# JiehongLin/SAM-6D

Measured on NVIDIA H100. Metric: poses/sec, higher is better.
Workload: dtype bf16

## Files before the change

include/sam6d_b200.h:

```cpp
#ifndef SAM6D_B200_H
#define SAM6D_B200_H

#ifdef __cplusplus
extern "C" {
#endif


int sam6d_fps(const float* xyz, int b, int n, int m, float* temp, int* idx, void* stream);
int sam6d_fps_single_cta(const float* xyz, int b, int n, int m, float* temp, int* idx, void* stream);

int sam6d_gather_points(const float* points, const int* idx, int b, int c, int n, int m, float* out, void* stream);

int sam6d_gather_rows(const float* src, const int* idx, int b, int n, int m, int c, long long src_bstride, float* out,
                      void* stream);
int sam6d_gather_rows_bf16_f32(const void* src, const int* idx, int b, int n, int m, int c, long long src_bstride, float* out,
                               void* stream);

int sam6d_ball_query(const float* new_xyz, const float* xyz, int b, int n, int m, float radius, int nsample, int* idx,
                     int* cnt, void* stream);
int sam6d_ball_query_pair(const float* new_xyz, const float* xyz, int b, int n, int m, float radius_a, int nsample_a,
                          float radius_b, int nsample_b, int* idx_a, int* idx_b, int* cnt_a, int* cnt_b, void* stream);

int sam6d_group_points(const float* points, const int* idx, int b, int c, int n, int np, int ns, float* out, void* stream);

// ... 43 lines not shown
                        const float* bias, float* E, void* stream);

int sam6d_geo_embed_tc(const float* T, long long npairs, const float* div_term, const void* Wa_bf16, const void* Wd_bf16,
                       const float* bias, void* E, int e_is_bf16, void* stream);
int sam6d_geo_embed_dist_tc(const float* T, long long npairs, const float* div_term, const void* Wd_bf16, const float* bias, void* E,
                            void* stream);
int sam6d_geo_embed_lut(const float* T, long long clouds, int S, const void* tabA, int na, float inv_ha, const void* tabD, int nd,
                        float inv_hd, const void* far, const float* div_term, const void* WdT_bf16, const float* bias, void* E,
                        int precise, void* stream);


int sam6d_inputs_stage_a(const int* rle_cum, const int* rle_off, int P, int H, int W, const float* depth, double fx, double fy,
                         double cx, double cy, double thr, unsigned char* mask, int* stats, int cap, int* choose1, int* choose2,
                         float* cloud2, void* stream);
int sam6d_inputs_stage_b(const int* stats, const int* keep, int Q, int H, int W, int cap, const int* choose2, const float* cloud2,
                         const int* choose_idx, int ns, int S, const unsigned char* image, const unsigned char* mask, int mask_flag,
                         float* pts, long long* rgb_choose, float* rgb, unsigned char* rgb_u8, void* stream);

int sam6d_crop_resize_normalize(const unsigned char* images, const unsigned char* masks, const int* bbox, int Q, int H, int W, int S,
                                int mask_flag, float* rgb, unsigned char* rgb_u8, void* stream);


int sam6d_crop_resize_pad(const unsigned char* image, const float* masks, const int* boxes, int P, int H, int W, int T, float* rgb,
                          float* pmask, void* stream);
int sam6d_masked_patch_normalize(const float* tokens, long long tok_ld, long long tok_bs, const float* pmask, int P, int G, int patch,
                                 int C, float thresh, float* out_f32, void* out_bf16, unsigned char* valid, void* stream);
int sam6d_appearance_reduce(const float* sim, long long sim_ld, long long sim_bs, int P, int N, const unsigned char* qvalid, float thred,
                            float* appe, float* vis, void* stream);


int sam6d_query_translation(const float* masks, const int* depth, int N, int H, int W, const double* K, double depth_scale,
                            float* translate, void* stream);
int sam6d_project_template_iou(const float* poses, int T, const float* pointcloud, int O, int npc, const long long* best_pose,
                               const long long* pred_obj, const float* translate, const double* K, int N, int H, int W,
                               const long long* boxes, int* image_vu, int* xyxy, float* iou, unsigned char* ok, void* stream);


int sam6d_sam_pe_encode(const float* coords, const float* G, int rows, float* out, void* stream);
int sam6d_sam_self_attn(const float* q, const float* k, const float* v, int B, int T, float* out, void* stream);
int sam6d_sam_tok2img_attn(const float* Q, const void* K, const void* V, long long kv_bs, int B, int T, int L, float* out, void* stream);
int sam6d_sam_img2tok_attn(const void* Q, long long q_bs, const float* Kt, const float* Vt, int B, int T, int L, void* out, void* stream);
int sam6d_sam_ln2d_gelu(const void* x, const float* gamma, const float* beta, long long rows, void* y, void* stream);
int sam6d_sam_mask_dot(const void* up, const float* hyper, int B, int G, float* masks, void* stream);
int sam6d_sam_mask_stats(const float* low, int N, int S, int big, int in_h, int in_w, int H, int W, float thr, float off, int* stats,
                         void* stream);
int sam6d_sam_mask_binarize(const float* low, const int* sel, int K, int S, int big, int in_h, int in_w, int H, int W, float thr,
                            unsigned char* out, void* stream);
int sam6d_sam_nms(const float* boxes, int N, float thr, unsigned char* keep, void* stream);


int sam6d_transformer_tail_bf16(const void* hid, long long ld_hid, const void* x, long long ld_x, const void* Wo, const float* bo,
                                const float* g1, const float* b1, const void* We, const float* be, const void* Ws, const float* bs,
                                const float* g2, const float* b2, void* out, long long ld_out, int M, float eps, void* stream);


int sam6d_rpe_scores(const void* E, int e_is_bf16, const float* U, long long u_ld, int B, int S, float* SP, void* stream);
int sam6d_rpe_scores_tc(const void* E, const void* U, int B, int S, float* SP, void* stream);
int sam6d_rpe_scores_tc_ld(const void* E, const void* U, int B, int S, float* SP, int sp_ld, void* stream);
int sam6d_mha(const float* Q, long long q_ld, long long q_bs, const float* K, long long k_ld, long long k_bs, const float* V,
              long long v_ld, long long v_bs, const float* bias, int B, int H, int Sq, int Sk, float scale, float* O,
              long long o_ld, long long o_bs, void* stream);
int sam6d_attn_tc(const void* Q, long long q_ld, int q_col0, const void* K, long long k_ld, int k_col0, const void* Vt,
                  long long vt_ld, int B, int H, int Sq, int Sk, int head_dim, int bias_mode, const float* bias,
                  const void* rel_h, const float* rel_w, int Hs, int Ws, const float* bv, float scale, void* out,
                  int out_is_bf16, long long out_ld, void* stream);
int sam6d_attn_tc_bias_ld(const void* Q, long long q_ld, int q_col0, const void* K, long long k_ld, int k_col0, const void* Vt,
                          long long vt_ld, int B, int H, int Sq, int Sk, int head_dim, const float* bias, long long bias_ld,
                          float scale, void* out, int out_is_bf16, long long out_ld, void* stream);
int sam6d_attn_tc_ex(const void* Q, long long q_ld, int q_col0, const void* K, long long k_ld, int k_col0, const void* Vt,
                     long long vt_ld, int B, int H, int Sq, int Sk, int head_dim, float scale, int k_brows, int k_row0, int v_col0,
                     float* lse, void* out, int out_is_bf16, long long out_ld, void* stream);
int sam6d_attn_merge_key(const void* Q, long long q_ld, int q_col0, const void* K, long long k_ld, int k_col0, int k_brows,
                         int key_row, const void* Vt, long long vt_ld, int key_col, const float* lse, int B, int H, int Sq,
                         float scale, void* out, long long out_ld, void* stream);
int sam6d_transpose_tokens_bf16(const void* src, long long ld, int col0, int C, int nB, int L, int N1, void* out, void* stream);
int sam6d_linattn_kv(const float* Kf, long long k_ld, long long k_bs, const float* V, long long v_ld, long long v_bs, int B,
                     int H, int J, float* KV, float* KS, void* stream);
int sam6d_linattn_apply(const float* Qf, long long q_rpb, long long q_bs, long long q_ld, const float* KV, const float* KS,
                        int B, int H, float* X, long long x_bs, long long x_ld, void* stream);
int sam6d_linattn_kv_pack(const float* Kf, long long k_ld, long long k_bs, const float* V, long long v_ld, long long v_bs, int B,
                          int J, void* blob, float* KS, void* stream);
int sam6d_linattn_tc(const void* Q, long long q_ld, long long q_bs, const void* blob, const float* KS,
                     const float* softplus_scale, int B, int rpb, void* X, long long x_ld, long long x_bs, void* stream);

int sam6d_coarse_assign(const float* A, int B, int S, float* W, float* w1, void* stream);
int sam6d_coarse_sample(const float* W, int B, int L, const float* rand, int nr, int* idx, void* stream);
int sam6d_coarse_hypotheses(const int* idx, const float* pts1, const float* pts2, int B, int n, int n1, float* Rt,
                            float* resid, void* stream);
int sam6d_topk_smallest(const float* v, int B, int n, int k, int* out, void* stream);
int sam6d_coarse_select(const float* Rt, const int* top, int B, int n1, int n2, const float* pts1, const float* w1, int n,
                        const float* model, int nm, float* scores, float* R, float* t, void* stream);


int sam6d_pe_mlp_max(const float* pts, const int* idx, const int* cnt, int B, int N, int ns, const float* W1,
                     const float* B1, const float* W2, const float* B2, const float* W3, const float* B3, float* out,
                     int out_ld, int out_off, void* stream);
int sam6d_pe_mlp_max_tc(const float* pts, const int* idx, int B, int N, int ns, const float* W1, const float* B1,
                        const void* W2_bf16, const float* B2, const void* W3_bf16, const float* B3, void* out, int out_is_bf16,
                        int out_ld, int out_off, void* stream);
int sam6d_fine_assign(const float* A, int B, int S, int ld, float shift, const float* pts2, float* rsum, float* csum, float* cpart,
                      int* cpi, int* lab1, int* lab2, float* wts, float* pred, void* stream);
int sam6d_fine_pass_tc(const void* Fa, const void* Fb, int B, int S, float alpha, float shift, int mode, const float* row_f,
                       const float* col_f, int ld_f, const float* q4, float* out_inv, int* lab, float* wts, float* pred, void* stream);
int sam6d_fine_masked_points(const int* lab2, const float* pts2, int B, int S, int ld, float* q4, void* stream);
int sam6d_weighted_procrustes(const float* src, const float* ref, const float* wts, int B, int N, float weight_thresh,
                              float eps, float* R, float* t, void* stream);
int sam6d_pose_score(const float* pts1, const int* lab1, int B, int N, const float* R, const float* t, const float* model,
                     int nm, float dis_thres, const float* radius, float* score, float* t_scaled, void* stream);

int sam6d_bilinear_gather(const void* up, int up_is_bf16, const long long* choose, int B, int K, int G, int sub, int C, int H, int W,
                          float* out, void* stream);

int sam6d_attn_relpos(const float* qkv, long long tok_ld, int nW, int Hs, int Ws, int nH, int head_dim, const float* rel_h,
                      const float* rel_w, float scale, void* out, int out_is_bf16, long long out_ld, void* stream);

int sam6d_attn_global_tc(const void* qkv, long long ld, const void* Vt, long long vt_ld, const void* rel_blob, int B, int H, int grid,
                         float scale, void* out, int out_is_bf16, long long out_ld, void* stream);

int sam6d_template_score(const float* Qn, const float* Rn, int P, int O, int T, int C, float* sim_out, float* obj_score,
                         int* best_obj, float* best_score, int* best_tmpl, void* stream);

const char* sam6d_version(void);

#ifdef __cplusplus
}
#endif
#endif
```

sam6d_b200/ops.py:

```python
import ctypes
from typing import Optional, Tuple

import torch

from . import _lib

Tensor = torch.Tensor


def _check(t: Tensor, dtype, name: str, ndim: Optional[int] = None):
    if not isinstance(t, torch.Tensor):
        raise RuntimeError(f"{name} must be a torch.Tensor")
    if not t.is_cuda:
        raise RuntimeError(f"{name} must be a CUDA tensor (CPU not supported)")
    if t.dtype != dtype:
        raise RuntimeError(f"{name} must be {dtype}, got {t.dtype}")
    if not t.is_contiguous():
        raise RuntimeError(f"{name} must be contiguous")
    if ndim is not None and t.dim() != ndim:
        raise RuntimeError(f"{name} must have {ndim} dims, got {t.dim()}")


def _p(t: Optional[Tensor]):
    return ctypes.c_void_p(0 if t is None else t.data_ptr())
# ... 466 lines not shown

def attn_global_tc(qkv: Tensor, vt: Tensor, rel_blob: Tensor, B: int, H: int, grid: int, scale: float, out_dtype=torch.bfloat16) -> Tensor:
    _check(qkv, torch.bfloat16, "qkv", 2)
    _check(vt, torch.bfloat16, "vt", 2)
    _check(rel_blob, torch.bfloat16, "rel_blob", 1)
    L = grid * grid
    out = torch.empty(B * L, H * 80, dtype=out_dtype, device=qkv.device)
    _lib.call("sam6d_attn_global_tc", _p(qkv), _ll(qkv.shape[1]), _p(vt), _ll(vt.shape[1]), _p(rel_blob), int(B), int(H), int(grid),
              _f(scale), _p(out), int(out_dtype == torch.bfloat16), _ll(H * 80), _s())
    return out


def attn_tc(Q: Tensor, q_col0: int, K: Tensor, k_col0: int, Vt: Tensor, B: int, H: int, Sq: int, Sk: int, D: int, scale: float,
            bias: Optional[Tensor] = None, rel: Optional[tuple] = None, bv: Optional[Tensor] = None,
            out_dtype=torch.float32, bias_variant: int = 1) -> Tensor:
    _check(Q, torch.bfloat16, "Q", 2)
    _check(K, torch.bfloat16, "K", 2)
    _check(Vt, torch.bfloat16, "Vt", 2)
    mode, rh, rw, Hs, Ws = 0, None, None, 0, 0
    if bias is not None:
        _check(bias, torch.float32, "bias", 4)
        mode = bias_variant
    elif rel is not None:
        rh, Hs, Ws = rel
        mode = 2
    out = torch.empty(B * Sq, H * D, dtype=out_dtype, device=Q.device)
    _lib.call("sam6d_attn_tc", _p(Q), _ll(Q.shape[1]), int(q_col0), _p(K), _ll(K.shape[1]), int(k_col0), _p(Vt), _ll(Vt.shape[1]),
              int(B), int(H), int(Sq), int(Sk), int(D), mode, _p(bias), _p(rh), _p(rw), int(Hs), int(Ws), _p(bv), _f(scale), _p(out),
              int(out_dtype == torch.bfloat16), _ll(H * D), _s())
    return out


def attn_tc_ex(Q: Tensor, q_col0: int, K: Tensor, k_col0: int, Vt: Tensor, B: int, H: int, Sq: int, Sk: int, D: int, scale: float,
               k_brows: int, k_row0: int = 0, v_col0: int = 0, want_lse: bool = False, out_dtype=torch.bfloat16):
    _check(Q, torch.bfloat16, "Q", 2)
    _check(K, torch.bfloat16, "K", 2)
    _check(Vt, torch.bfloat16, "Vt", 2)
    out = torch.empty(B * Sq, H * D, dtype=out_dtype, device=Q.device)
    lse = torch.empty(B, H, Sq, dtype=torch.float32, device=Q.device) if want_lse else None
    _lib.call("sam6d_attn_tc_ex", _p(Q), _ll(Q.shape[1]), int(q_col0), _p(K), _ll(K.shape[1]), int(k_col0), _p(Vt), _ll(Vt.shape[1]),
              int(B), int(H), int(Sq), int(Sk), int(D), _f(scale), int(k_brows), int(k_row0), int(v_col0), _p(lse), _p(out),
              int(out_dtype == torch.bfloat16), _ll(H * D), _s())
    return out, lse


def attn_merge_key(Q: Tensor, q_col0: int, K: Tensor, k_col0: int, k_brows: int, key_row: int, Vt: Tensor, key_col: int, lse: Tensor,
                   B: int, H: int, Sq: int, scale: float, out: Tensor) -> Tensor:
    _check(out, torch.bfloat16, "out", 2)
    _check(lse, torch.float32, "lse", 3)
    _lib.call("sam6d_attn_merge_key", _p(Q), _ll(Q.shape[1]), int(q_col0), _p(K), _ll(K.shape[1]), int(k_col0), int(k_brows), int(key_row),
              _p(Vt), _ll(Vt.shape[1]), int(key_col), _p(lse), int(B), int(H), int(Sq), _f(scale), _p(out), _ll(out.shape[1]), _s())
    return out


def transpose_tokens(src: Tensor, col0: int, C: int, nB: int, L: int) -> Tensor:
    _check(src, torch.bfloat16, "src", 2)
    N1 = (L + 15) // 16 * 16
    out = torch.empty(nB * C, N1, dtype=torch.bfloat16, device=src.device)
    _lib.call("sam6d_transpose_tokens_bf16", _p(src), _ll(src.shape[1]), int(col0), int(C), int(nB), int(L), int(N1), _p(out), _s())
    return out


def linattn_kv_raw(k_ptr, k_ld, k_bs, v_ptr, v_ld, v_bs, B, H, J, KV: Tensor, KS: Tensor):
    _lib.call("sam6d_linattn_kv", ctypes.c_void_p(k_ptr), _ll(k_ld), _ll(k_bs), ctypes.c_void_p(v_ptr), _ll(v_ld), _ll(v_bs),
              int(B), int(H), int(J), _p(KV), _p(KS), _s())


def linattn_apply_raw(q_ptr, q_rpb, q_bs, q_ld, KV: Tensor, KS: Tensor, B, H, x_ptr, x_bs, x_ld):
    _lib.call("sam6d_linattn_apply", ctypes.c_void_p(q_ptr), _ll(q_rpb), _ll(q_bs), _ll(q_ld), _p(KV), _p(KS), int(B), int(H),
              ctypes.c_void_p(x_ptr), _ll(x_bs), _ll(x_ld), _s())


def linattn_kv_pack_raw(k_ptr, k_ld, k_bs, v_ptr, v_ld, v_bs, B, J, device):
    blob = torch.empty(B, 4 * 64 * 64, dtype=torch.bfloat16, device=device)
    KS = torch.empty(B, 4, 64, dtype=torch.float32, device=device)
    _lib.call("sam6d_linattn_kv_pack", ctypes.c_void_p(k_ptr), _ll(k_ld), _ll(k_bs), ctypes.c_void_p(v_ptr), _ll(v_ld), _ll(v_bs),
              int(B), int(J), _p(blob), _p(KS), _s())
    return blob, KS


def linattn_tc_raw(q_ptr, q_ld, q_bs, blob: Tensor, KS: Tensor, sp_scale: Tensor, B, rpb, x_ptr, x_ld, x_bs):
    _lib.call("sam6d_linattn_tc", ctypes.c_void_p(q_ptr), _ll(q_ld), _ll(q_bs), _p(blob), _p(KS), _p(sp_scale), int(B), int(rpb),
              ctypes.c_void_p(x_ptr), _ll(x_ld), _ll(x_bs), _s())


def coarse_assign(A: Tensor) -> Tuple[Tensor, Tensor]:
    _check(A, torch.float32, "atten", 3)
    B, S, _ = A.shape
    n = S - 1
    W = torch.empty(B, n * n, dtype=torch.float32, device=A.device)
    w1 = torch.empty(B, n, dtype=torch.float32, device=A.device)
    _lib.call("sam6d_coarse_assign", _p(A), B, S, _p(W), _p(w1), _s())
    return W, w1


def coarse_sample(W: Tensor, rand: Tensor) -> Tensor:
    _check(W, torch.float32, "W", 2)
    _check(rand, torch.float32, "rand", 2)
    B, L = W.shape
    nr = rand.shape[1]
    idx = torch.empty(B, nr, dtype=torch.int32, device=W.device)
    _lib.call("sam6d_coarse_sample", _p(W), B, L, _p(rand), nr, _p(idx), _s())
    return idx


def coarse_hypotheses(idx: Tensor, pts1: Tensor, pts2: Tensor) -> Tuple[Tensor, Tensor]:
    _check(idx, torch.int32, "idx", 2)
    _check(pts1, torch.float32, "pts1", 3)
    _check(pts2, torch.float32, "pts2", 3)
    B, n, _ = pts1.shape
    n1 = idx.shape[1] // 3
    Rt = torch.empty(B, n1, 12, dtype=torch.float32, device=idx.device)
    resid = torch.empty(B, n1, dtype=torch.float32, device=idx.device)
    _lib.call("sam6d_coarse_hypotheses", _p(idx), _p(pts1), _p(pts2), B, n, n1, _p(Rt), _p(resid), _s())
    return Rt, resid


def topk_smallest(v: Tensor, k: int) -> Tensor:
    _check(v, torch.float32, "v", 2)
    B, n = v.shape
    out = torch.empty(B, k, dtype=torch.int32, device=v.device)
    _lib.call("sam6d_topk_smallest", _p(v), B, n, int(k), _p(out), _s())
    return out


def coarse_select(Rt: Tensor, top: Tensor, pts1: Tensor, w1: Tensor, model: Tensor):
    _check(Rt, torch.float32, "Rt", 3)
    _check(top, torch.int32, "top", 2)
    _check(model, torch.float32, "model", 3)
    B, n1, _ = Rt.shape
    n2 = top.shape[1]
    n = pts1.shape[1]
    scores = torch.empty(B, n2, dtype=torch.float32, device=Rt.device)
    R = torch.empty(B, 3, 3, dtype=torch.float32, device=Rt.device)
    t = torch.empty(B, 3, dtype=torch.float32, device=Rt.device)
    _lib.call("sam6d_coarse_select", _p(Rt), _p(top), B, n1, n2, _p(pts1), _p(w1), n, _p(model), model.shape[1], _p(scores),
              _p(R), _p(t), _s())
    return R, t, scores


def pe_mlp_max(pts: Tensor, idx: Tensor, cnt: Tensor, weights, out: Tensor, out_off: int):
    _check(pts, torch.float32, "pts", 3)
    _check(idx, torch.int32, "idx", 3)
    _check(cnt, torch.int32, "cnt", 2)
    B, N, _ = pts.shape
    ns = idx.shape[2]
    W1, B1, W2, B2, W3, B3 = weights
    _lib.call("sam6d_pe_mlp_max", _p(pts), _p(idx), _p(cnt), B, N, ns, _p(W1), _p(B1), _p(W2), _p(B2), _p(W3), _p(B3),
              _p(out), out.shape[-1], int(out_off), _s())


def pe_mlp_max_tc(pts: Tensor, idx: Tensor, weights, out: Tensor, out_off: int):
    _check(pts, torch.float32, "pts", 3)
    _check(idx, torch.int32, "idx", 3)
    B, N, _ = pts.shape
    ns = idx.shape[2]
    W1, B1, W2, B2, W3, B3 = weights
    _check(W2, torch.bfloat16, "W2", 2)
    _check(W3, torch.bfloat16, "W3", 2)
    if out.dtype not in (torch.float32, torch.bfloat16):
        raise RuntimeError("pe_mlp_max_tc: out must be float32 or bfloat16")
    _lib.call("sam6d_pe_mlp_max_tc", _p(pts), _p(idx), B, N, ns, _p(W1), _p(B1), _p(W2), _p(B2), _p(W3), _p(B3), _p(out),
              int(out.dtype == torch.bfloat16), out.shape[-1], int(out_off), _s())


def fine_assign(A: Tensor, pts2: Tensor, shift: float):
# ... 118 lines not shown
```

sam6d_b200/pem.py:

```python
import math
import os
from types import SimpleNamespace
from typing import Dict, Optional

import torch
import torch.nn as nn

from . import ops

NUM_HEADS = 4

PRECISIONS = ("fp32", "bf16")
FUSED_TAIL = os.environ.get("SAM6D_FUSED_TAIL", "1") != "0"
PADDED_BIAS = os.environ.get("SAM6D_PADDED_BIAS", "1") != "0"
RPE_TC = os.environ.get("SAM6D_RPE_TC", "1") != "0"
GEO_LUT = os.environ.get("SAM6D_GEO_LUT", "1") != "0"
GEO_LUT_PRECISE = os.environ.get("SAM6D_GEO_LUT_PRECISE", "1") != "0"
GEO_LUT_INV_H = 8.0
GEO_LUT_D_MAX = 32.0


class _W:
    __slots__ = ("f32", "bf16")

    def __init__(self, w: torch.Tensor):
        self.f32 = w.detach().to(torch.float32).contiguous()
        self.bf16 = self.f32.to(torch.bfloat16).contiguous()


def _gemm(prec, A, W: "_W", bias=None, residual=None, relu=False):
    if prec == "bf16":
        if A.dtype == torch.bfloat16 and residual is None and A.is_contiguous() and A.shape[1] % 64 == 0:
            return ops.gemm_tma(A, W.bf16, bias, act=1 if relu else 0)
        return ops.gemm_tc(A, W.bf16, bias, residual=residual, relu=relu)
    return ops.gemm(A, W.f32, bias, residual=residual, relu=relu)


def _gemm_raw(prec, A_ptr, W: "_W", bias, R_ptr, C_ptr, M, N, K, lda, ldc, ldr=0, batch=1, sA=0, sC=0, sR=0):
    if prec == "bf16":
        ops.gemm_tc_raw(A_ptr, 0, W.bf16.data_ptr(), 1, bias, R_ptr, C_ptr, 0, M, N, K, lda, K, ldc, ldr, batch=batch, sA=sA, sW=0,
                        sC=sC, sR=sR)
    else:
        ops.gemm_raw(A_ptr, W.f32.data_ptr(), bias, R_ptr, C_ptr, M, N, K, lda, K, ldc, ldr, batch=batch, sA=sA, sW=0, sC=sC, sR=sR)


def _cfg(cfg, **defaults):
    if isinstance(cfg, dict):
        cfg = SimpleNamespace(**cfg)
    for k, v in defaults.items():
        if not hasattr(cfg, k):
            setattr(cfg, k, v)
    return cfg


class _MHAParams(nn.Module):
    def __init__(self, d_model, rpe: bool):
        super().__init__()
        self.proj_q = nn.Linear(d_model, d_model)
        self.proj_k = nn.Linear(d_model, d_model)
        self.proj_v = nn.Linear(d_model, d_model)
        if rpe:
            self.proj_p = nn.Linear(d_model, d_model)


class _AttentionLayerParams(nn.Module):
    def __init__(self, d_model, rpe: bool):
        super().__init__()
        self.attention = _MHAParams(d_model, rpe)
        self.linear = nn.Linear(d_model, d_model)
        self.norm = nn.LayerNorm(d_model)


class _AttentionOutputParams(nn.Module):
    def __init__(self, d_model):
        super().__init__()
        self.expand = nn.Linear(d_model, d_model * 2)
        self.squeeze = nn.Linear(d_model * 2, d_model)
        self.norm = nn.LayerNorm(d_model)


class _TransformerLayerParams(nn.Module):
    def __init__(self, d_model, rpe: bool):
        super().__init__()
        self.attention = _AttentionLayerParams(d_model, rpe)
        self.output = _AttentionOutputParams(d_model)


class _Packed:

    def __init__(self):
        self.key = None
        self.w = {}


def _param_key(module: nn.Module):
    return tuple((p.data_ptr(), p._version) for p in module.parameters()) + tuple(
# ... 450 lines not shown
                ops.pe_mlp_max_tc(pts, idx, w[name + "_tc"], feat, off)
            else:
                ops.pe_mlp_max(pts, idx, cnt, w[name], feat, off)
        return feat

    @torch.no_grad()
    def forward(self, pts1, pts2=None):
        if pts2 is not None and pts2 is not pts1:
            raise NotImplementedError("SAM-6D always calls PE(pts) with a single cloud")
        w = self._weights()
        feat = self.local_features(pts1)
        B, N, _ = feat.shape
        if self.precision == "bf16":
            return ops.gemm_tma(feat.view(B * N, 256), w["w3"].bf16, w["b3"]).view(B, N, -1)
        return _gemm(self.precision, feat.view(B * N, 256), w["w3"], w["b3"]).view(B, N, -1)


class _LinearAttentionParams(nn.Module):
    def __init__(self, d_model):
        super().__init__()
        self.proj_q = nn.Linear(d_model, d_model)
        self.proj_k = nn.Linear(d_model, d_model)
        self.proj_v = nn.Linear(d_model, d_model)
        self.scale = nn.Parameter(torch.zeros(size=(1, 1, d_model)))


class _LinearAttentionLayerParams(nn.Module):
    def __init__(self, d_model):
        super().__init__()
        self.attention = _LinearAttentionParams(d_model)
        self.linear = nn.Linear(d_model, d_model)
        self.norm = nn.LayerNorm(d_model)


class _LinearTransformerLayerParams(nn.Module):
    def __init__(self, d_model):
        super().__init__()
        self.attention = _LinearAttentionLayerParams(d_model)
        self.output = _AttentionOutputParams(d_model)


class SparseToDenseTransformer(nn.Module):

    def __init__(self, d_model, sparse_blocks, num_heads=4, dropout=None, activation_fn='ReLU', parallel=False,
                 focusing_factor=3, with_bg_token=True, replace_bg_token=True):
        super().__init__()
        if not (with_bg_token and replace_bg_token) or focusing_factor != 3:
            raise ValueError("sam6d_b200 SparseToDenseTransformer is built for the SAM-6D configuration")
        self.d_model = d_model
        self.sparse_layer = GeometricTransformer(blocks=sparse_blocks, d_model=d_model, num_heads=num_heads, dropout=dropout,
                                                 activation_fn=activation_fn, parallel=parallel, return_attention_scores=False)
        self.dense_layer = _LinearTransformerLayerParams(d_model)
        self._packed = _Packed()
        self.precision = "fp32"

    def _weights(self):
        key = _param_key(self.dense_layer)
        if self._packed.key != key:
            la = self.dense_layer.attention.attention
            tail = dict(wo=_W(self.dense_layer.attention.linear.weight), bo=_f32(self.dense_layer.attention.linear.bias),
                        g1=_f32(self.dense_layer.attention.norm.weight), b1=_f32(self.dense_layer.attention.norm.bias),
                        we=_W(self.dense_layer.output.expand.weight), be=_f32(self.dense_layer.output.expand.bias),
                        ws=_W(self.dense_layer.output.squeeze.weight), bs=_f32(self.dense_layer.output.squeeze.bias),
                        g2=_f32(self.dense_layer.output.norm.weight), b2=_f32(self.dense_layer.output.norm.bias))
            self._packed.w = dict(
                wq=_W(la.proj_q.weight), bq=_f32(la.proj_q.bias),
                wkv=_W(torch.cat([_f32(la.proj_k.weight), _f32(la.proj_v.weight)], dim=0)),
                bkv=torch.cat([_f32(la.proj_k.bias), _f32(la.proj_v.bias)], dim=0).contiguous(),
                sp_scale=torch.nn.functional.softplus(_f32(la.scale)).reshape(-1).contiguous(), tail=tail)
            self._packed.key = key
        return self._packed.w

    def _sample_feats(self, dense_feats, idx_ext):
        if dense_feats.dtype == torch.bfloat16:
            return ops.gather_rows_bf16(dense_feats, idx_ext)
        return ops.gather_rows(dense_feats, idx_ext)

    def _dense_layer_bf16(self, dense, sparse, w):
        B, N1, C = dense.shape
        N, J = N1 - 1, sparse.shape[1] - 1
        dev = dense.device
        bf = torch.bfloat16
        x2d = dense.view(B * N1, C)
        q = ops.gemm_tma(x2d, w["wq"].bf16, w["bq"], out_dtype=bf)
        kv = torch.empty(B * J, 2 * C, dtype=torch.float32, device=dev)
        s_bf = sparse.dtype == torch.bfloat16
        ops.gemm_tc_raw(sparse.data_ptr() + C * (2 if s_bf else 4), int(s_bf), w["wkv"].bf16.data_ptr(), 1, w["bkv"], 0, kv.data_ptr(), 0,
                        J, 2 * C, C, C, C, 2 * C, 0, batch=B, sA=(J + 1) * C, sW=0, sC=J * 2 * C)
        ops.focus_rows_raw(kv.data_ptr(), (B * J, 0, 2 * C), kv.data_ptr(), (B * J, 0, 2 * C), w["sp_scale"], B * J, C)
        blob, KS = ops.linattn_kv_pack_raw(kv.data_ptr(), 2 * C, J * 2 * C, kv.data_ptr() + C * 4, 2 * C, J * 2 * C, B, J, dev)
        x_att = torch.empty(B * N1, C, dtype=bf, device=dev)
        ops.linattn_tc_raw(q.data_ptr() + C * 2, C, N1 * C, blob, KS, w["sp_scale"], B, N, x_att.data_ptr() + C * 2, C, N1 * C)
        x_att.view(B, N1, C)[:, 0, :] = 0
        t = w["tail"]
        if FUSED_TAIL:
            out = ops.transformer_tail_bf16(x_att, x2d, t["wo"].bf16, t["bo"], t["g1"], t["b1"], t["we"].bf16, t["be"], t["ws"].bf16,
                                            t["bs"], t["g2"], t["b2"]).view(B, N1, C)
        else:
            y = ops.gemm_tma(x_att, t["wo"].bf16, t["bo"], residual=x2d, out_dtype=bf)
            y = ops.layernorm_bf16io(y, t["g1"], t["b1"])
            h = ops.gemm_tma(y, t["we"].bf16, t["be"], act=1, out_dtype=bf)
            z = ops.gemm_tma(h, t["ws"].bf16, t["bs"], residual=y, out_dtype=bf)
            out = ops.layernorm_bf16io(z, t["g2"], t["b2"]).view(B, N1, C)
        out[:, 0, :] = sparse[:, 0, :].to(bf)
        return out

    def _dense_layer(self, dense, sparse, w):
        B, N1, C = dense.shape
        N, J = N1 - 1, sparse.shape[1] - 1
        f = 4
        dev = dense.device
        x_ptr, x_view = dense.data_ptr() + C * f, (N, N1 * C, C)
        q = torch.empty(B * N, C, dtype=torch.float32, device=dev)
        prec = self.precision
        _gemm_raw(prec, x_ptr, w["wq"], w["bq"], 0, q.data_ptr(), N, C, C, C, C, 0, batch=B, sA=N1 * C, sC=N * C)
        kv = torch.empty(B * J, 2 * C, dtype=torch.float32, device=dev)
        _gemm_raw(prec, sparse.data_ptr() + C * f, w["wkv"], w["bkv"], 0, kv.data_ptr(), J, 2 * C, C, C, 2 * C, 0, batch=B,
                  sA=(J + 1) * C, sC=J * 2 * C)
        ops.focus_rows_raw(q.data_ptr(), (B * N, 0, C), q.data_ptr(), (B * N, 0, C), w["sp_scale"], B * N, C)
        ops.focus_rows_raw(kv.data_ptr(), (B * J, 0, 2 * C), kv.data_ptr(), (B * J, 0, 2 * C), w["sp_scale"], B * J, C)
        KV = torch.empty(B, NUM_HEADS, 64, 64, dtype=torch.float32, device=dev)
        KS = torch.empty(B, NUM_HEADS, 64, dtype=torch.float32, device=dev)
        ops.linattn_kv_raw(kv.data_ptr(), 2 * C, J * 2 * C, kv.data_ptr() + C * f, 2 * C, J * 2 * C, B, NUM_HEADS, J, KV, KS)
        x_att = torch.empty(B * N, C, dtype=torch.float32, device=dev)
        ops.linattn_apply_raw(q.data_ptr(), N, N * C, C, KV, KS, B, NUM_HEADS, x_att.data_ptr(), N * C, C)
        t = w["tail"]
        y = torch.empty(B * N, C, dtype=torch.float32, device=dev)
        _gemm_raw(prec, x_att.data_ptr(), t["wo"], t["bo"], x_ptr, y.data_ptr(), N, C, C, C, C, C, batch=B, sA=N * C, sC=N * C,
                  sR=N1 * C)
        y = ops.layernorm(y, t["g1"], t["b1"])
        h = _gemm(prec, y, t["we"], t["be"], relu=True)
        z = _gemm(prec, h, t["ws"], t["bs"], residual=y)
        out = torch.empty(B, N1, C, dtype=torch.float32, device=dev)
        ops.layernorm_raw(z.data_ptr(), (B * N, 0, C), out.data_ptr() + C * f, (N, N1 * C, C), t["g2"], t["b2"], B * N, C)
        out[:, 0, :] = sparse[:, 0, :]
        return out

    @torch.no_grad()
    def forward(self, dense_feats0, embeddings0, fps_idx0, dense_feats1, embeddings1, fps_idx1, masks0=None, masks1=None):
        w = self._weights()
        ext0 = torch.cat([torch.zeros_like(fps_idx0[:, :1]), fps_idx0], dim=1).contiguous()
        ext1 = torch.cat([torch.zeros_like(fps_idx1[:, :1]), fps_idx1], dim=1).contiguous()
        dense = _stack2(dense_feats0, dense_feats1)
        if dense is not None:
            B = dense_feats0.shape[0]
            feats = self._sample_feats(dense, torch.cat([ext0, ext1], dim=0))
            feats0, feats1 = self.sparse_layer(feats[:B], embeddings0, feats[B:], embeddings1, masks0, masks1)
            layer = self._dense_layer_bf16 if dense.dtype == torch.bfloat16 else self._dense_layer
            out = layer(dense, torch.cat([feats0, feats1], dim=0), w)
            return out[:B], out[B:]
        feats0 = self._sample_feats(dense_feats0.contiguous(), ext0)
        feats1 = self._sample_feats(dense_feats1.contiguous(), ext1)
        feats0, feats1 = self.sparse_layer(feats0, embeddings0, feats1, embeddings1, masks0, masks1)
        layer = self._dense_layer_bf16 if dense_feats0.dtype == torch.bfloat16 else self._dense_layer
        dense_feats0 = layer(dense_feats0.contiguous(), feats0, w)
        dense_feats1 = layer(dense_feats1.contiguous(), feats1, w)
        return dense_feats0, dense_feats1


class FinePointMatching(nn.Module):

    def __init__(self, cfg, return_feat=False):
        super().__init__()
        self.cfg = _cfg(cfg)
        self.return_feat = return_feat
        self.nblock = self.cfg.nblock
        self.in_proj = nn.Linear(self.cfg.input_dim, self.cfg.hidden_dim)
        self.out_proj = nn.Linear(self.cfg.hidden_dim, self.cfg.out_dim)
        self.bg_token = nn.Parameter(torch.randn(1, 1, self.cfg.hidden_dim) * .02)
        self.PE = PositionalEncoding(self.cfg.hidden_dim, r1=self.cfg.pe_radius1, r2=self.cfg.pe_radius2)
        self._packed = _Packed()
        self.precision = "fp32"
        self.transformers = nn.ModuleList([
# ... 189 lines not shown
```

Before: 2577.

## Fuse dense linear-attention layer into one persistent warp-specialized WGMMA kernel

Adds a single persistent kernel that computes, per 128-row tile, the Q projection, the focused linear-attention feature map and apply, the output projection with LayerNorm, the FFN, and the second LayerNorm. A TMA producer warpgroup streams the weights through a 3-stage ring. It replaces a Q GEMM, the linattn_tc kernel, the zeroing of row 0, the fused tail and the background-row copy. The aim is to remove launches and the global-memory round trips of the intermediate activations. In exchange it adds a complex kernel hardcoded to C=256 and hidden=512, with large register and shared-memory use.

```diff
diff --git a/include/sam6d_b200.h b/include/sam6d_b200.h
--- a/include/sam6d_b200.h
+++ b/include/sam6d_b200.h
@@ -149,6 +149,10 @@
                           int J, void* blob, float* KS, void* stream);
 int sam6d_linattn_tc(const void* Q, long long q_ld, long long q_bs, const void* blob, const float* KS,
                      const float* softplus_scale, int B, int rpb, void* X, long long x_ld, long long x_bs, void* stream);
+int sam6d_dense_linattn_layer_bf16(const void* x, const void* Wq, const float* bq, const void* blob, const float* KS,
+                                   const float* softplus_scale, const void* Wo, const float* bo, const float* g1, const float* b1,
+                                   const void* We, const float* be, const void* Ws, const float* bs, const float* g2, const float* b2,
+                                   const void* bg, int bg_bf16, long long bg_bs, void* out, int B, int N, float eps, void* stream);
 
 int sam6d_coarse_assign(const float* A, int B, int S, float* W, float* w1, void* stream);
 int sam6d_coarse_sample(const float* W, int B, int L, const float* rand, int nr, int* idx, void* stream);
diff --git a/sam6d_b200/csrc/dense_layer_tc.cu b/sam6d_b200/csrc/dense_layer_tc.cu
--- /dev/null
+++ b/sam6d_b200/csrc/dense_layer_tc.cu
@@ -0,0 +1,352 @@
+#include <cuda.h>
+
+#include "tc.cuh"
+
+namespace {
+
+constexpr int BM = 128, C = 256, HID = 512, BK = 64, H = 4, D = 64;
+constexpr int T_SLAB = BM * 128;
+constexpr int T_BYTES = 4 * T_SLAB;
+constexpr int W_STAGE = 256 * 128;
+constexpr int B_SLAB = 64 * 128;
+constexpr int W_STAGES = 3;
+constexpr int W_PER_TILE = 25;
+constexpr int CONSUMERS = 256, THREADS = CONSUMERS + 128;
+constexpr int SMEM = 2 * T_BYTES + W_STAGES * W_STAGE + 1024;
+
+struct LayerArgs {
+  const float* bq; const float* bo; const float* g1; const float* b1;
+  const float* be; const float* bs; const float* g2; const float* b2;
+  const uint8_t* blob; const float* KS; const float* sp_scale;
+  const void* bg; int bg_bf16; long long bg_bs;
+  __nv_bfloat16* out;
+  int B, N, tiles_per_cloud;
+  float eps;
+};
+
+__device__ __forceinline__ uint32_t* tile_pair(uint8_t* tile, int r, int col) {
+  return reinterpret_cast<uint32_t*>(tile + (col >> 6) * T_SLAB + r * 128 + ((((col & 63) >> 3) ^ (r & 7)) << 4) + (col & 7) * 2);
+}
+__device__ __forceinline__ float2 unpack2(uint32_t w) { return make_float2(__uint_as_float(w << 16), __uint_as_float(w & 0xffff0000u)); }
+
+__device__ __forceinline__ void tma_load_3d(const void* tmap, uint64_t* bar, void* smem_dst, int c0, int c1, int c2) {
+  asm volatile("cp.async.bulk.tensor.3d.shared::cluster.global.mbarrier::complete_tx::bytes [%0], [%1, {%3, %4, %5}], [%2];" ::"r"(
+                   tc::smem_u32(smem_dst)),
+               "l"(reinterpret_cast<uint64_t>(tmap)), "r"(tc::smem_u32(bar)), "r"(c0), "r"(c1), "r"(c2)
+               : "memory");
+}
+
+__global__ void __launch_bounds__(THREADS, 1) dense_layer_tc_kernel(const __grid_constant__ CUtensorMap tmX, const __grid_constant__ CUtensorMap tmWq,
+                                                       const __grid_constant__ CUtensorMap tmWo, const __grid_constant__ CUtensorMap tmWe,
+                                                       const __grid_constant__ CUtensorMap tmWs, LayerArgs a) {
+  extern __shared__ __align__(1024) uint8_t smem_raw[];
+  uint8_t* smem = reinterpret_cast<uint8_t*>((reinterpret_cast<uintptr_t>(smem_raw) + 1023) & ~(uintptr_t)1023);
+  uint8_t* a_buf = smem;
+  uint8_t* x_buf = smem + T_BYTES;
+  uint8_t* w_ring = smem + 2 * T_BYTES;
+  __shared__ __align__(8) uint64_t in_full, in_empty, w_full[W_STAGES], w_empty[W_STAGES];
+
+  const int tid = threadIdx.x, warp = tid >> 5, lane = tid & 31;
+  const int ntiles = a.B * a.tiles_per_cloud;
+  const long long cloud_rows = a.N + 1;
+
+  if (tid == 0) {
+    tc::mbar_init(&in_full, 1); tc::mbar_init(&in_empty, CONSUMERS / 32);
+    for (int s = 0; s < W_STAGES; ++s) { tc::mbar_init(&w_full[s], 1); tc::mbar_init(&w_empty[s], CONSUMERS / 32); }
+    tc::mbar_fence_init();
+    tc::tma_prefetch_desc(&tmX); tc::tma_prefetch_desc(&tmWq); tc::tma_prefetch_desc(&tmWo);
+    tc::tma_prefetch_desc(&tmWe); tc::tma_prefetch_desc(&tmWs);
+  }
+  s6_pdl_trigger();
+  __syncthreads();
+  s6_pdl_wait();
+
+  if (warp >= CONSUMERS / 32) {
+    tc::producer_regs();
+    if (tid == CONSUMERS) {
+      long long gw = 0;
+      int it = 0;
+      for (int tile = blockIdx.x; tile < ntiles; tile += gridDim.x, ++it) {
+        const int b = tile / a.tiles_per_cloud, row0 = 1 + (tile - b * a.tiles_per_cloud) * BM;
+        auto load_w = [&](int j) {
+          const int s = (int)(gw % W_STAGES);
+          tc::mbar_wait(&w_empty[s], (uint32_t)(((gw / W_STAGES) & 1) ^ 1));
+          tc::mbar_arrive_expect_tx(&w_full[s], W_STAGE);
+          uint8_t* dst = w_ring + s * W_STAGE;
+          if (j < 4) tc::tma_load_2d(&tmWq, &w_full[s], dst, j * BK, 0);
+          else if (j == 4) tc::bulk_load_1d(dst, a.blob + (size_t)b * W_STAGE, W_STAGE, &w_full[s]);
+          else if (j < 9) tc::tma_load_2d(&tmWo, &w_full[s], dst, (j - 5) * BK, 0);
+          else if (j < 17) tc::tma_load_2d(&tmWe, &w_full[s], dst, ((j - 9) & 3) * BK, ((j - 9) >> 2) * 256);
+          else tc::tma_load_2d(&tmWs, &w_full[s], dst, (j - 17) * BK, 0);
+          ++gw;
+        };
+        int j = 0;
+        for (; j < W_STAGES; ++j) load_w(j);
+        tc::mbar_wait(&in_empty, (uint32_t)((it & 1) ^ 1));
+        tc::mbar_arrive_expect_tx(&in_full, T_BYTES);
+#pragma unroll
+        for (int kb = 0; kb < 4; ++kb) tma_load_3d(&tmX, &in_full, x_buf + kb * T_SLAB, kb * BK, row0, b);
+        for (; j < W_PER_TILE; ++j) load_w(j);
+      }
+    }
+    return;
+  }
+  tc::consumer_regs();
+  for (int b = blockIdx.x; b < a.B; b += gridDim.x) {
+    __nv_bfloat16* o = a.out + (size_t)b * cloud_rows * C + tid;
+    if (a.bg_bf16) *o = reinterpret_cast<const __nv_bfloat16*>(a.bg)[(size_t)b * a.bg_bs + tid];
+    else *o = __float2bfloat16(reinterpret_cast<const float*>(a.bg)[(size_t)b * a.bg_bs + tid]);
+  }
+  const int wg = warp >> 2, w = warp & 3;
+  const uint32_t a_addr = tc::smem_u32(a_buf) + wg * (64 * 128), x_addr = tc::smem_u32(x_buf) + wg * (64 * 128), w_addr0 = tc::smem_u32(w_ring);
+  long long gw = 0;
+  float acc[C / 2];
+  auto gemm = [&](uint32_t op_addr, uint32_t op_addr2, int nkb) {
+    int prev = -1;
+    for (int kb = 0; kb < nkb; ++kb, ++gw) {
+      const int s = (int)(gw % W_STAGES);
+      tc::mbar_wait(&w_full[s], (uint32_t)((gw / W_STAGES) & 1));
+      const uint32_t op = (kb < 4 ? op_addr : op_addr2) + (kb & 3) * T_SLAB;
+      tc::wg_fence();
+#pragma unroll
+      for (int k = 0; k < 4; ++k)
+        tc::wgmma_bf16<C>(acc, tc::wg_desc(op + k * 32), tc::wg_desc(w_addr0 + s * W_STAGE + k * 32), (kb | k) ? 1u : 0u);
+      tc::wg_commit();
+      if (prev >= 0) {
+        tc::wg_wait<1>();
+        if (lane == 0) tc::mbar_arrive(&w_empty[prev]);
+      }
+      prev = s;
+    }
+    tc::wg_wait<0>();
+    if (lane == 0) tc::mbar_arrive(&w_empty[prev]);
+  };
+  auto layernorm = [&](const float* __restrict__ bias, const float* __restrict__ g, const float* __restrict__ b, auto&& residual) {
+    float s[2] = {0.f, 0.f}, q[2] = {0.f, 0.f};
+#pragma unroll
+    for (int e = 0; e < C / 2; e += 2) {
+      const int hr = (e >> 1) & 1, col = tc::frag_col(e, lane);
+      const float2 bb = __ldg(reinterpret_cast<const float2*>(bias + col)), rr = residual(e, hr, col);
+      acc[e] += bb.x + rr.x; acc[e + 1] += bb.y + rr.y;
+      s[hr] += acc[e] + acc[e + 1];
+      q[hr] = fmaf(acc[e], acc[e], fmaf(acc[e + 1], acc[e + 1], q[hr]));
+    }
+    float mean[2], rstd[2];
+#pragma unroll
+    for (int hr = 0; hr < 2; ++hr) {
+      mean[hr] = tc::quad_sum(s[hr]) * (1.f / C);
+      rstd[hr] = rsqrtf(fmaxf(tc::quad_sum(q[hr]) * (1.f / C) - mean[hr] * mean[hr], 0.f) + a.eps);
+    }
+#pragma unroll
+    for (int e = 0; e < C / 2; e += 2) {
+      const int hr = (e >> 1) & 1, col = tc::frag_col(e, lane);
+      const float2 gg = __ldg(reinterpret_cast<const float2*>(g + col)), bb = __ldg(reinterpret_cast<const float2*>(b + col));
+      acc[e] = fmaf((acc[e] - mean[hr]) * rstd[hr], gg.x, bb.x);
+      acc[e + 1] = fmaf((acc[e + 1] - mean[hr]) * rstd[hr], gg.y, bb.y);
+    }
+  };
+  auto relu_store = [&](const float* __restrict__ bias, uint8_t* dst) {
+#pragma unroll
+    for (int e = 0; e < C / 2; e += 2) {
+      const int col = tc::frag_col(e, lane), r = wg * 64 + tc::frag_row(e, w, lane);
+      const float2 bb = __ldg(reinterpret_cast<const float2*>(bias + col));
+      *tile_pair(dst, r, col) = tc::pack_bf16(fmaxf(acc[e] + bb.x, 0.f), fmaxf(acc[e + 1] + bb.y, 0.f));
+    }
+  };
+  auto publish = [&]() {
+    tc::fence_proxy_async_smem();
+    tc::named_bar(1 + wg, 128);
+  };
+  const int head = lane >> 3, piece = lane & 7;
+  int it = 0;
+  for (int tile = blockIdx.x; tile < ntiles; tile += gridDim.x, ++it) {
+    const int b = tile / a.tiles_per_cloud, t0 = (tile - b * a.tiles_per_cloud) * BM;
+    __nv_bfloat16* ob = a.out + ((size_t)b * cloud_rows + 1) * C;
+    tc::mbar_wait(&in_full, (uint32_t)(it & 1));
+    gemm(x_addr, x_addr, 4);
+#pragma unroll
+    for (int e = 0; e < C / 2; e += 2) {
+      const int r = wg * 64 + tc::frag_row(e, w, lane), col = tc::frag_col(e, lane);
+      const float2 bb = __ldg(reinterpret_cast<const float2*>(a.bq + col));
+      *tile_pair(a_buf, r, col) = tc::pack_bf16(acc[e] + bb.x, acc[e + 1] + bb.y);
+    }
+    tc::named_bar(1 + wg, 128);
+    float rs[8], ksv[8];
+    {
+      const float4 s0 = *reinterpret_cast<const float4*>(a.sp_scale + lane * 8), s1 = *reinterpret_cast<const float4*>(a.sp_scale + lane * 8 + 4);
+      rs[0] = 1.f / s0.x; rs[1] = 1.f / s0.y; rs[2] = 1.f / s0.z; rs[3] = 1.f / s0.w;
+      rs[4] = 1.f / s1.x; rs[5] = 1.f / s1.y; rs[6] = 1.f / s1.z; rs[7] = 1.f / s1.w;
+      const float4 k0 = *reinterpret_cast<const float4*>(a.KS + (size_t)b * C + lane * 8), k1 = *reinterpret_cast<const float4*>(a.KS + (size_t)b * C + lane * 8 + 4);
+      ksv[0] = k0.x; ksv[1] = k0.y; ksv[2] = k0.z; ksv[3] = k0.w; ksv[4] = k1.x; ksv[5] = k1.y; ksv[6] = k1.z; ksv[7] = k1.w;
+    }
+    float z[2][H] = {};
+#pragma unroll 1
+    for (int i0 = 0; i0 < 16; i0 += 4) {
+      const int rbase = wg * 64 + w * 16 + i0;
+      uint4 raw[4];
+#pragma unroll
+      for (int u = 0; u < 4; ++u) {
+        const int r = rbase + u;
+        raw[u] = *reinterpret_cast<const uint4*>(a_buf + head * T_SLAB + r * 128 + ((piece ^ (r & 7)) << 4));
+      }
+#pragma unroll
+      for (int u = 0; u < 4; ++u) {
+        const int r = rbase + u, i = i0 + u;
+        const uint32_t wd[4] = {raw[u].x, raw[u].y, raw[u].z, raw[u].w};
+        float q[8];
+        float s1 = 0.f, s3 = 0.f;
+#pragma unroll
+        for (int e = 0; e < 4; ++e) {
+          q[2 * e] = __uint_as_float(wd[e] << 16);
+          q[2 * e + 1] = __uint_as_float(wd[e] & 0xffff0000u);
+        }
+#pragma unroll
+        for (int e = 0; e < 8; ++e) {
+          float tt = (fmaxf(q[e], 0.f) + 1e-6f) * rs[e];
+          s1 = fmaf(tt, tt, s1);
+          tt = tt * tt * tt;
+          s3 = fmaf(tt, tt, s3);
+          q[e] = tt;
+        }
+        s1 = warp_sum(s1);
+        s3 = warp_sum(s3);
+        const float n = sqrtf(s1) * rsqrtf(s3);
+        float zp = 0.f;
+#pragma unroll
+        for (int e = 0; e < 8; ++e) { q[e] *= n; zp = fmaf(q[e], ksv[e], zp); }
+        zp += __shfl_xor_sync(0xffffffffu, zp, 1);
+        zp += __shfl_xor_sync(0xffffffffu, zp, 2);
+        zp += __shfl_xor_sync(0xffffffffu, zp, 4);
+        const float zinv = 1.f / (zp + 1e-6f);
+#pragma unroll
+        for (int h = 0; h < H; ++h) {
+          const float v = __shfl_sync(0xffffffffu, zinv, h * 8);
+          if (i == (lane >> 2)) z[0][h] = v;
+          if (i == (lane >> 2) + 8) z[1][h] = v;
+        }
+        *reinterpret_cast<uint4*>(a_buf + head * T_SLAB + r * 128 + ((piece ^ (r & 7)) << 4)) =
+            make_uint4(tc::pack_bf16(q[0], q[1]), tc::pack_bf16(q[2], q[3]), tc::pack_bf16(q[4], q[5]), tc::pack_bf16(q[6], q[7]));
+      }
+    }
+    publish();
+    {
+      const int s = (int)(gw % W_STAGES);
+      tc::mbar_wait(&w_full[s], (uint32_t)((gw / W_STAGES) & 1));
+      const uint32_t b_addr = w_addr0 + s * W_STAGE;
+      float(&acc_h)[D / 2] = *reinterpret_cast<float(*)[D / 2]>(acc);
+#pragma unroll
+      for (int h = 0; h < H; ++h) {
+        tc::wg_fence();
+#pragma unroll
+        for (int k = 0; k < D / 16; ++k)
+          tc::wgmma_bf16<D>(acc_h, tc::wg_desc(a_addr + h * T_SLAB + k * 32), tc::wg_desc(b_addr + h * B_SLAB + k * 32), k ? 1u : 0u);
+        tc::wg_commit();
+        tc::wg_wait<0>();
+        if (h == H - 1 && lane == 0) tc::mbar_arrive(&w_empty[s]);
+#pragma unroll
+        for (int hr = 0; hr < 2; ++hr) {
+          const int r = wg * 64 + tc::frag_row(2 * hr, w, lane);
+#pragma unroll
+          for (int jj = 0; jj < D / 8; ++jj)
+            *tile_pair(a_buf, r, h * D + tc::frag_col(4 * jj, lane)) =
+                tc::pack_bf16(acc_h[4 * jj + 2 * hr] * z[hr][h], acc_h[4 * jj + 2 * hr + 1] * z[hr][h]);
+        }
+      }
+      ++gw;
+    }
+    publish();
+    gemm(a_addr, a_addr, 4);
+    layernorm(a.bo, a.g1, a.b1, [&](int e, int hr, int col) {
+      return unpack2(*tile_pair(x_buf, wg * 64 + tc::frag_row(e, w, lane), col));
+    });
+#pragma unroll
+    for (int e = 0; e < C / 2; e += 2) {
+      const int r = wg * 64 + tc::frag_row(e, w, lane), col = tc::frag_col(e, lane), row = t0 + r;
+      const uint32_t y2 = tc::pack_bf16(acc[e], acc[e + 1]);
+      *tile_pair(a_buf, r, col) = y2;
+      if (row < a.N) *reinterpret_cast<uint32_t*>(ob + (size_t)row * C + col) = y2;
+    }
+    publish();
+    gemm(a_addr, a_addr, 4);
+    relu_store(a.be, x_buf);
+    gemm(a_addr, a_addr, 4);
+    tc::named_bar(1 + wg, 128);
+    relu_store(a.be + 256, a_buf);
+    publish();
+    gemm(x_addr, a_addr, 8);
+    if (lane == 0) tc::mbar_arrive(&in_empty);
+    layernorm(a.bs, a.g2, a.b2, [&](int e, int, int col) {
+      const int row = t0 + wg * 64 + tc::frag_row(e, w, lane);
+      return row < a.N ? unpack2(*reinterpret_cast<const uint32_t*>(ob + (size_t)row * C + col)) : make_float2(0.f, 0.f);
+    });
+#pragma unroll
+    for (int e = 0; e < C / 2; e += 2) {
+      const int row = t0 + wg * 64 + tc::frag_row(e, w, lane);
+      if (row < a.N) *reinterpret_cast<uint32_t*>(ob + (size_t)row * C + tc::frag_col(e, lane)) = tc::pack_bf16(acc[e], acc[e + 1]);
+    }
+  }
+}
+
+typedef CUresult (*EncodeFn)(CUtensorMap*, CUtensorMapDataType, cuuint32_t, void*, const cuuint64_t*, const cuuint64_t*,
+                             const cuuint32_t*, const cuuint32_t*, CUtensorMapInterleave, CUtensorMapSwizzle,
+                             CUtensorMapL2promotion, CUtensorMapFloatOOBfill);
+
+EncodeFn get_encode() {
+  static EncodeFn fn = nullptr;
+  if (!fn) {
+    void* p = nullptr;
+    cudaDriverEntryPointQueryResult q;
+    if (cudaGetDriverEntryPoint("cuTensorMapEncodeTiled", &p, cudaEnableDefault, &q) != cudaSuccess || q != cudaDriverEntryPointSuccess)
+      return nullptr;
+    fn = reinterpret_cast<EncodeFn>(p);
+  }
+  return fn;
+}
+
+int make_map(CUtensorMap* map, const void* ptr, int rank, long long planes, long long rows, long long cols, int box_rows) {
+  EncodeFn enc = get_encode();
+  if (!enc) return 999;
+  cuuint64_t gdim[3] = {(cuuint64_t)cols, (cuuint64_t)rows, (cuuint64_t)planes};
+  cuuint64_t gstride[2] = {(cuuint64_t)cols * 2, (cuuint64_t)(rows * cols * 2)};
+  cuuint32_t box[3] = {64, (cuuint32_t)box_rows, 1};
+  cuuint32_t estr[3] = {1, 1, 1};
+  CUresult r = enc(map, CU_TENSOR_MAP_DATA_TYPE_BFLOAT16, (cuuint32_t)rank, const_cast<void*>(ptr), gdim, gstride, box, estr,
+                   CU_TENSOR_MAP_INTERLEAVE_NONE, CU_TENSOR_MAP_SWIZZLE_128B, CU_TENSOR_MAP_L2_PROMOTION_L2_256B,
+                   CU_TENSOR_MAP_FLOAT_OOB_FILL_NONE);
+  return r == CUDA_SUCCESS ? 0 : 1000 + (int)r;
+}
+
+}
+
+S6_API int sam6d_dense_linattn_layer_bf16(const void* x, const void* Wq, const float* bq, const void* blob, const float* KS,
+                                          const float* softplus_scale, const void* Wo, const float* bo, const float* g1,
+                                          const float* b1, const void* We, const float* be, const void* Ws, const float* bs,
+                                          const float* g2, const float* b2, const void* bg, int bg_bf16, long long bg_bs, void* out,
+                                          int B, int N, float eps, void* stream) {
+  S6_REQUIRE(x && Wq && bq && blob && KS && softplus_scale && Wo && bo && g1 && b1 && We && be && Ws && bs && g2 && b2 && bg && out);
+  S6_REQUIRE(B >= 0 && N >= 1 && bg_bs >= C && (long long)B * (N + 1) < 2000000000LL);
+  S6_REQUIRE(((reinterpret_cast<uintptr_t>(x) | reinterpret_cast<uintptr_t>(out) | reinterpret_cast<uintptr_t>(blob) |
+               reinterpret_cast<uintptr_t>(Wq) | reinterpret_cast<uintptr_t>(Wo) | reinterpret_cast<uintptr_t>(We) |
+               reinterpret_cast<uintptr_t>(Ws) | reinterpret_cast<uintptr_t>(KS) | reinterpret_cast<uintptr_t>(softplus_scale) |
+               reinterpret_cast<uintptr_t>(bq) | reinterpret_cast<uintptr_t>(bo) | reinterpret_cast<uintptr_t>(be) |
+               reinterpret_cast<uintptr_t>(bs) | reinterpret_cast<uintptr_t>(g1) | reinterpret_cast<uintptr_t>(b1) |
+               reinterpret_cast<uintptr_t>(g2) | reinterpret_cast<uintptr_t>(b2)) & 15) == 0);
+  if (B == 0) return 0;
+  CUtensorMap tmX, tmWq, tmWo, tmWe, tmWs;
+  int rc;
+  if ((rc = make_map(&tmX, x, 3, B, N + 1, C, BM))) return rc;
+  if ((rc = make_map(&tmWq, Wq, 2, 1, C, C, 256))) return rc;
+  if ((rc = make_map(&tmWo, Wo, 2, 1, C, C, 256))) return rc;
+  if ((rc = make_map(&tmWe, We, 2, 1, HID, C, 256))) return rc;
+  if ((rc = make_map(&tmWs, Ws, 2, 1, C, HID, 256))) return rc;
+  int dev = 0, sms = 0;
+  S6_CHECK(cudaGetDevice(&dev));
+  S6_CHECK(cudaDeviceGetAttribute(&sms, cudaDevAttrMultiProcessorCount, dev));
+  const int tpc = s6_cdiv(N, BM), ntiles = B * tpc, grid = ntiles < sms ? ntiles : sms;
+  LayerArgs a{bq, bo, g1, b1, be, bs, g2, b2, reinterpret_cast<const uint8_t*>(blob), KS, softplus_scale, bg, bg_bf16, bg_bs,
+              reinterpret_cast<__nv_bfloat16*>(out), B, N, tpc, eps};
+  S6_CHECK(cudaFuncSetAttribute(dense_layer_tc_kernel, cudaFuncAttributeMaxDynamicSharedMemorySize, SMEM));
+  S6_CHECK(s6_launch_pdl(dense_layer_tc_kernel, dim3(grid), dim3(THREADS), SMEM, s6_stream(stream), tmX, tmWq, tmWo, tmWe, tmWs, a));
+  S6_LAUNCH_CHECK();
+  return 0;
+}
diff --git a/sam6d_b200/ops.py b/sam6d_b200/ops.py
--- a/sam6d_b200/ops.py
+++ b/sam6d_b200/ops.py
@@ -572,6 +572,30 @@
 def linattn_tc_raw(q_ptr, q_ld, q_bs, blob: Tensor, KS: Tensor, sp_scale: Tensor, B, rpb, x_ptr, x_ld, x_bs):
     _lib.call("sam6d_linattn_tc", ctypes.c_void_p(q_ptr), _ll(q_ld), _ll(q_bs), _p(blob), _p(KS), _p(sp_scale), int(B), int(rpb),
               ctypes.c_void_p(x_ptr), _ll(x_ld), _ll(x_bs), _s())
+
+
+def dense_linattn_layer_bf16(x: Tensor, wq: Tensor, bq: Tensor, blob: Tensor, KS: Tensor, sp_scale: Tensor, tail: dict, bg: Tensor,
+                             out: Optional[Tensor] = None, eps: float = 1e-5) -> Tensor:
+    _check(x, torch.bfloat16, "x", 3)
+    B, N1, C = x.shape
+    if C != 256 or N1 < 2 or bg.dim() != 3 or bg.shape[0] != B or bg.shape[2] != C or bg.dtype not in _DT or not bg.is_contiguous():
+        raise RuntimeError("dense_linattn_layer_bf16: x (B,N+1,256) bf16, bg (B,J+1,256) contiguous fp32 | bf16")
+    for w, shape in ((wq, (256, 256)), (tail["wo"].bf16, (256, 256)), (tail["we"].bf16, (512, 256)), (tail["ws"].bf16, (256, 512))):
+        _check(w, torch.bfloat16, "weight", 2)
+        if tuple(w.shape) != shape:
+            raise RuntimeError("dense_linattn_layer_bf16: d_model 256, hidden 512")
+    _check(blob, torch.bfloat16, "blob", 2)
+    _check(KS, torch.float32, "KS", 3)
+    if blob.shape != (B, 4 * 64 * 64) or KS.shape != (B, 4, 64):
+        raise RuntimeError("dense_linattn_layer_bf16: blob (B, 16384), KS (B, 4, 64)")
+    if out is None:
+        out = torch.empty_like(x)
+    _check(out, torch.bfloat16, "out", 3)
+    t = tail
+    _lib.call("sam6d_dense_linattn_layer_bf16", _p(x), _p(wq), _p(bq), _p(blob), _p(KS), _p(sp_scale), _p(t["wo"].bf16), _p(t["bo"]),
+              _p(t["g1"]), _p(t["b1"]), _p(t["we"].bf16), _p(t["be"]), _p(t["ws"].bf16), _p(t["bs"]), _p(t["g2"]), _p(t["b2"]), _p(bg),
+              _DT[bg.dtype], _ll(bg.shape[1] * C), _p(out), int(B), int(N1 - 1), _f(eps), _s())
+    return out
 
 
 def coarse_assign(A: Tensor) -> Tuple[Tensor, Tensor]:
diff --git a/sam6d_b200/pem.py b/sam6d_b200/pem.py
--- a/sam6d_b200/pem.py
+++ b/sam6d_b200/pem.py
@@ -12,6 +12,7 @@
 
 PRECISIONS = ("fp32", "bf16")
 FUSED_TAIL = os.environ.get("SAM6D_FUSED_TAIL", "1") != "0"
+FUSED_DENSE = os.environ.get("SAM6D_FUSED_DENSE", "1") != "0"
 PADDED_BIAS = os.environ.get("SAM6D_PADDED_BIAS", "1") != "0"
 RPE_TC = os.environ.get("SAM6D_RPE_TC", "1") != "0"
 GEO_LUT = os.environ.get("SAM6D_GEO_LUT", "1") != "0"
@@ -628,13 +629,15 @@
         dev = dense.device
         bf = torch.bfloat16
         x2d = dense.view(B * N1, C)
-        q = ops.gemm_tma(x2d, w["wq"].bf16, w["bq"], out_dtype=bf)
         kv = torch.empty(B * J, 2 * C, dtype=torch.float32, device=dev)
         s_bf = sparse.dtype == torch.bfloat16
         ops.gemm_tc_raw(sparse.data_ptr() + C * (2 if s_bf else 4), int(s_bf), w["wkv"].bf16.data_ptr(), 1, w["bkv"], 0, kv.data_ptr(), 0,
                         J, 2 * C, C, C, C, 2 * C, 0, batch=B, sA=(J + 1) * C, sW=0, sC=J * 2 * C)
         ops.focus_rows_raw(kv.data_ptr(), (B * J, 0, 2 * C), kv.data_ptr(), (B * J, 0, 2 * C), w["sp_scale"], B * J, C)
         blob, KS = ops.linattn_kv_pack_raw(kv.data_ptr(), 2 * C, J * 2 * C, kv.data_ptr() + C * 4, 2 * C, J * 2 * C, B, J, dev)
+        if FUSED_DENSE:
+            return ops.dense_linattn_layer_bf16(dense, w["wq"].bf16, w["bq"], blob, KS, w["sp_scale"], w["tail"], sparse)
+        q = ops.gemm_tma(x2d, w["wq"].bf16, w["bq"], out_dtype=bf)
         x_att = torch.empty(B * N1, C, dtype=bf, device=dev)
         ops.linattn_tc_raw(q.data_ptr() + C * 2, C, N1 * C, blob, KS, w["sp_scale"], B, N, x_att.data_ptr() + C * 2, C, N1 * C)
         x_att.view(B, N1, C)[:, 0, :] = 0
```

Result: faster. 2666 (median of 6 runs) (+3.5%).
